# ooowedyn/InkLayer

Hardware: AMD Instinct MI355X
Metric: sketches/sec end-to-end (GroundingDINO+SAM) at 1024x1024 (higher is better)
Workload: dtype f16 (MFMA, f32 accumulate; f32 residual/norm/softmax; split-f16 = fp32-grade operands for patch-embed, neck, mask decoder)

## Files before the change

inklayer_amd/csrc/gemm.hip:

```cpp
#include <stdlib.h>

#include "common.h"
#include "../../include/inklayer_hip.h"

namespace {

template <int BK> struct Swz;
template <> struct Swz<64> {
  static __device__ __forceinline__ int f(int row) { return row & 7; }
};
template <> struct Swz<32> {
  static __device__ __forceinline__ int f(int row) { return (-(row >> 2)) & 3; }
};

typedef __attribute__((address_space(1))) const void* gptr_t;
typedef __attribute__((address_space(3))) void* lptr_t;

__device__ __forceinline__ bool residual_preloaded(const InkGemm& p) {
  return (p.residual || p.res_hi) && p.act == INK_ACT_NONE && !p.col_scale;
}

template <int TM>
__device__ __forceinline__ void wave_rows(int (&rows)[TM], const InkGemm& p, int mw, int lane) {
#pragma unroll
  for (int ti = 0; ti < TM; ++ti) {
    const int m = mw + ti * 16 + (lane & 15);
    int r = -1;
    if (m < p.M) r = p.row_map ? p.row_map[m] : m;
    rows[ti] = r;
  }
}

template <int TM, int TN, bool SPLIT = false>
__device__ __forceinline__ void init_wave_tile(f32x4 (&acc)[TM][TN], const InkGemm& p, const int (&rows)[TM], int nw,
                                               int lane) {
  const int fq = lane >> 4;
  const bool pre = residual_preloaded(p);
  if (SPLIT) {
#pragma unroll
    for (int ti = 0; ti < TM; ++ti) {
      const int r = pre ? rows[ti] : -1;
      const size_t off = (size_t)max(r, 0) * p.ldr + nw + fq * 4;
#pragma unroll
      for (int j = 0; j < TN; ++j) {
        acc[ti][j] = (f32x4){0.f, 0.f, 0.f, 0.f};
        if (r >= 0 && nw + j * 16 + fq * 4 < p.N) {
          const f16x4 h = *(const f16x4*)((const f16*)p.res_hi + off + j * 16);
          const f16x4 l = *(const f16x4*)((const f16*)p.res_lo + off + j * 16);
          acc[ti][j] = (f32x4){(float)h[0] + (float)l[0], (float)h[1] + (float)l[1], (float)h[2] + (float)l[2],
                               (float)h[3] + (float)l[3]};
        }
      }
    }
    return;
  }
#pragma unroll
  for (int ti = 0; ti < TM; ++ti) {
    const int r = pre ? rows[ti] : -1;
    const float* rp = p.residual + (size_t)max(r, 0) * p.ldr + nw + fq * 4;
#pragma unroll
    for (int j = 0; j < TN; ++j) {
      acc[ti][j] = (f32x4){0.f, 0.f, 0.f, 0.f};
      if (r >= 0 && nw + j * 16 + fq * 4 < p.N) acc[ti][j] = *(const f32x4*)(rp + j * 16);
    }
  }
}

template <int TM, int TN>
__device__ __forceinline__ void ln_rows_prologue(const InkGemm& p, float2* strip, int mw, int nw, int lane) {
  float2* cols = strip + TM * 16;
  for (int c = lane; c < TN * 16; c += 64) {
    const int n = nw + c;
    cols[c] = n < p.N ? make_float2(p.ln_colsum[n], p.bias ? p.bias[n] : 0.f) : make_float2(0.f, 0.f);
  }
  constexpr int RPL = (TM * 16 + 63) / 64;
  f32x4 v[RPL][10];
#pragma unroll
  for (int q = 0; q < RPL; ++q) {
    const int r = lane + 64 * q, m = mw + r;
    const f32x4* sp = (const f32x4*)((const float2*)p.ln_stats + (size_t)min(m, p.M - 1) * p.ln_parts);
#pragma unroll
    for (int k = 0; k < 10; ++k) v[q][k] = 2 * k < p.ln_parts ? sp[k] : (f32x4){0.f, 0.f, 0.f, 0.f};
  }
#pragma unroll
  for (int q = 0; q < RPL; ++q) {
    const int r = lane + 64 * q;
    double s1 = 0.0, s2 = 0.0;
#pragma unroll
    for (int k = 0; k < 10; ++k) {
      s1 += (double)v[q][k][0] + (double)v[q][k][2];
      s2 += (double)v[q][k][1] + (double)v[q][k][3];
    }
    const double mean = s1 / (double)p.ln_dim;
    const double var = fmax(s2 / (double)p.ln_dim - mean * mean, 0.0);
    const float rstd = (float)(1.0 / sqrt(var + (double)p.ln_eps));
    if (r < TM * 16) strip[r] = mw + r < p.M ? make_float2(rstd, rstd * (float)mean) : make_float2(0.f, 0.f);
  }
}

template <int TM, int TN>
__device__ __forceinline__ void add_bias_wave_tile(f32x4 (&acc)[TM][TN], const InkGemm& p, int nw, int lane) {
  const int fq = lane >> 4;
#pragma unroll
  for (int j = 0; j < TN; ++j) {
    const int n = nw + j * 16 + fq * 4;
    f32x4 bv = (f32x4){0.f, 0.f, 0.f, 0.f};
    if (p.bias && n < p.N) bv = *(const f32x4*)(p.bias + n);
#pragma unroll
    for (int ti = 0; ti < TM; ++ti) acc[ti][j] += bv;
  }
}

template <int TM, int TN, int OUT, int MODE = -1, bool LNF = false>
__device__ __forceinline__ void store_wave_tile(f32x4 (&acc)[TM][TN], const InkGemm& p, char* er,
                                                const int (&rows)[TM], int nw, int lane, const float2* strip = nullptr) {
  constexpr bool F16O = OUT == 1;
  constexpr int WNC = TN * 16, EP = WNC * 4 + 16;
  constexpr int ES = OUT == 0 ? 4 : 8;
  constexpr int CPRW = WNC / ES;
  constexpr int NIT = (16 * CPRW + 63) / 64;
  const int fr = lane & 15, fq = lane >> 4;
  const bool wide16 = OUT != 0 && (p.ldc % 8 == 0);
  const bool res_late = MODE < 0 && p.residual && !residual_preloaded(p);
  const int act = MODE < 0 ? p.act : MODE;
  const bool scaled = MODE < 0 && p.col_scale != nullptr;
  int row_of[NIT], n_of[NIT];
#pragma unroll
  for (int it = 0; it < NIT; ++it) {
    const int c = it * 64 + lane;
    row_of[it] = c < 16 * CPRW ? c / CPRW : 16;
    n_of[it] = nw + (c % CPRW) * ES;
  }

  if (LNF) {
    const float2* cols = strip + TM * 16;
#pragma unroll
    for (int j = 0; j < TN; ++j) {
      const f32x4 c01 = *(const f32x4*)(cols + j * 16 + fq * 4);
      const f32x4 c23 = *(const f32x4*)(cols + j * 16 + fq * 4 + 2);
      const f32x4 sv = (f32x4){c01[0], c01[2], c23[0], c23[2]}, bv = (f32x4){c01[1], c01[3], c23[1], c23[3]};
#pragma unroll
      for (int ti = 0; ti < TM; ++ti) {
        const float2 mr = strip[ti * 16 + fr];
#pragma unroll
        for (int e = 0; e < 4; ++e) acc[ti][j][e] = fmaf(mr.x, acc[ti][j][e], fmaf(-mr.y, sv[e], bv[e]));
      }
      __builtin_amdgcn_sched_barrier(0);
    }
  } else {
    add_bias_wave_tile<TM, TN>(acc, p, nw, lane);
  }

#pragma unroll
  for (int ti = 0; ti < TM; ++ti) {
    float s1 = 0.f, s2 = 0.f;
#pragma unroll
    for (int j = 0; j < TN; ++j) {
      f32x4 v = acc[ti][j];
      if (act == INK_ACT_GELU) {
#pragma unroll
        for (int r = 0; r < 4; ++r) v[r] = gelu_erf(v[r]);
      } else if (act == INK_ACT_RELU) {
#pragma unroll
        for (int r = 0; r < 4; ++r) v[r] = fmaxf(v[r], 0.f);
      }
      if (scaled) {
        const int n = nw + j * 16 + fq * 4;
        if (n < p.N) v *= *(const f32x4*)(p.col_scale + n);
      }
      if (OUT == 2 && nw + j * 16 + fq * 4 < p.N) {
        s1 += (v[0] + v[1]) + (v[2] + v[3]);
        s2 += (v[0] * v[0] + v[1] * v[1]) + (v[2] * v[2] + v[3] * v[3]);
      }
      if (F16O) {
        *(f16x4*)(er + fr * EP + (j * 16 + fq * 4) * 2) = (f16x4){(f16)v[0], (f16)v[1], (f16)v[2], (f16)v[3]};
      } else {
        *(f32x4*)(er + fr * EP + (j * 16 + fq * 4) * 4) = v;
      }
    }
    if (OUT == 2 && p.stats_out) {
      s1 += __shfl_xor(s1, 16, 64);
      s2 += __shfl_xor(s2, 16, 64);
      s1 += __shfl_xor(s1, 32, 64);
      s2 += __shfl_xor(s2, 32, 64);
      if (fq == 0 && rows[ti] >= 0)
        ((float2*)p.stats_out)[(size_t)rows[ti] * p.stats_parts + nw / WNC] = make_float2(s1, s2);
    }
#pragma unroll
    for (int it = 0; it < NIT; ++it) {
      int r = __builtin_amdgcn_ds_bpermute((row_of[it] & 15) << 2, rows[ti]);
      if (row_of[it] >= 16 || n_of[it] >= p.N) r = -1;
      if (r >= 0) {
        const int c_n = n_of[it];
        const char* src = er + row_of[it] * EP + (c_n - nw) * (F16O ? 2 : 4);
        if (F16O) {
          f16x8 d = *(const f16x8*)src;
          f16* dst = (f16*)p.C + (size_t)r * p.ldc + c_n;
          if (res_late) {
            const float* rp = p.residual + (size_t)r * p.ldr + c_n;
#pragma unroll
            for (int e = 0; e < 8; ++e)
              if (c_n + e < p.N) d[e] = (f16)((float)d[e] + rp[e]);
          }
          if (wide16 && c_n + 8 <= p.N) {
            *(f16x8*)dst = d;
          } else {
            *(f16x4*)dst = (f16x4){d[0], d[1], d[2], d[3]};
            if (c_n + 8 <= p.N) *(f16x4*)(dst + 4) = (f16x4){d[4], d[5], d[6], d[7]};
          }
        } else if (OUT == 2) {
          const f32x4 d0 = *(const f32x4*)src, d1 = *(const f32x4*)(src + 16);
          f16x8 hi, lo;
#pragma unroll
          for (int e = 0; e < 4; ++e) {
            hi[e] = (f16)d0[e];
            lo[e] = (f16)(d0[e] - (float)hi[e]);
            hi[e + 4] = (f16)d1[e];
            lo[e + 4] = (f16)(d1[e] - (float)hi[e + 4]);
          }
          f16* dh = (f16*)p.C + (size_t)r * p.ldc + c_n;
          f16* dl = (f16*)p.C_lo + (size_t)r * p.ldc + c_n;
          if (wide16 && c_n + 8 <= p.N) {
            *(f16x8*)dh = hi;
            *(f16x8*)dl = lo;
          } else {
            *(f16x4*)dh = (f16x4){hi[0], hi[1], hi[2], hi[3]};
            *(f16x4*)dl = (f16x4){lo[0], lo[1], lo[2], lo[3]};
            if (c_n + 8 <= p.N) {
              *(f16x4*)(dh + 4) = (f16x4){hi[4], hi[5], hi[6], hi[7]};
              *(f16x4*)(dl + 4) = (f16x4){lo[4], lo[5], lo[6], lo[7]};
            }
          }
        } else {
          f32x4 d = *(const f32x4*)src;
          if (res_late) d += *(const f32x4*)(p.residual + (size_t)r * p.ldr + c_n);
          *(f32x4*)((float*)p.C + (size_t)r * p.ldc + c_n) = d;
        }
      }
    }
  }
}

__device__ __forceinline__ void tile_of(int id, int ntm, int ntn, int group_m, int& mt, int& nt) {
  if (group_m > 1) {
    const int per = group_m * ntn;
    const int first = (id / per) * group_m;
    const int gsz = min(ntm - first, group_m);
    mt = first + (id % per) % gsz;
    nt = (id % per) / gsz;
  } else {
    mt = id / ntn;
    nt = id % ntn;
  }
}

constexpr int NS = 2;
template <int BM, int BN, int BK, int WM, int WN, bool EXT>
__global__ __launch_bounds__(WM * WN * 64) void gemm_f16_nt(InkGemm p, int group_m) {
  constexpr int NT = WM * WN * 64;
  constexpr int CPR = BK / 8;
  constexpr int ROWB = BK * 2;
  constexpr int TILE_A = BM * ROWB, TILE_W = BN * ROWB;
  constexpr int STAGE = TILE_A + TILE_W;
  constexpr int IT_A = (BM * CPR) / NT, IT_W = (BN * CPR) / NT;
  constexpr int TM = BM / WM / 16, TN = BN / WN / 16;
  static_assert((BM * CPR) % NT == 0 && (BN * CPR) % NT == 0, "tile/threads mismatch");
  extern __shared__ __attribute__((aligned(16))) char smem[];

  const int tid = threadIdx.x;
  const int lane = tid & 63;
  const int wave = tid >> 6;
  const int wm = wave / WN, wn = wave % WN;

  const int ntn = (p.N + BN - 1) / BN;
  const int ntm = (p.M + BM - 1) / BM;
  int mt, nt;
  tile_of(xcd_remap(blockIdx.x, ntm * ntn), ntm, ntn, group_m, mt, nt);
  const int m0 = mt * BM;
  const int n0 = nt * BN;

  const f16* __restrict__ A = (const f16*)p.A;
  const f16* __restrict__ W = (const f16*)p.W;

  const f16* srcA[IT_A];
  const f16* srcW[IT_W];
#pragma unroll
  for (int it = 0; it < IT_A; ++it) {
    const int pch = it * NT + tid;
    const int row = pch / CPR;
    const int lch = (pch % CPR) ^ Swz<BK>::f(row);
    srcA[it] = A + (size_t)min(m0 + row, p.M - 1) * p.lda + lch * 8;
  }
#pragma unroll
  for (int it = 0; it < IT_W; ++it) {
    const int pch = it * NT + tid;
    const int row = pch / CPR;
    const int lch = (pch % CPR) ^ Swz<BK>::f(row);
    srcW[it] = W + (size_t)min(n0 + row, p.N - 1) * p.ldw + lch * 8;
  }

  auto stage = [&](int buf, int kt) {
    char* base = smem + buf * STAGE;
#pragma unroll
    for (int it = 0; it < IT_A; ++it)
      __builtin_amdgcn_global_load_lds((gptr_t)(srcA[it] + kt * BK), (lptr_t)(base + (it * NT + wave * 64) * 16), 16, 0, 0);
#pragma unroll
    for (int it = 0; it < IT_W; ++it)
      __builtin_amdgcn_global_load_lds((gptr_t)(srcW[it] + kt * BK), (lptr_t)(base + TILE_A + (it * NT + wave * 64) * 16), 16, 0, 0);
  };

  int rows[TM];
  wave_rows<TM>(rows, p, m0 + wm * (BM / WM), lane);
  f32x4 acc[TM][TN];
  float2* strip = (float2*)(smem + NS * STAGE) + wave * (TM * 16 + TN * 16);
  if (EXT && p.ln_stats) ln_rows_prologue<TM, TN>(p, strip, m0 + wm * (BM / WM), n0 + wn * (BN / WN), lane);

  const int fr = lane & 15, fq = lane >> 4;
  const int offA = (wm * (BM / WM) + fr) * ROWB;
  const int offW = (wn * (BN / WN) + fr) * ROWB;
  const int swz = Swz<BK>::f(fr);

  const int nk = p.K / BK;
  auto compute = [&](int cur) {
    const char* bA = smem + cur * STAGE;
    const char* bW = bA + TILE_A;
#pragma unroll
    for (int kk = 0; kk < BK / 32; ++kk) {
      constexpr int AG = TM > 4 ? 4 : TM;
      f16x8 a[AG], w[TN];
      const int co = ((kk * 4 + fq) ^ swz) << 4;
#pragma unroll
      for (int j = 0; j < TN; ++j) w[j] = *(const f16x8*)(bW + offW + j * 16 * ROWB + co);
#pragma unroll
      for (int i0 = 0; i0 < TM; i0 += AG) {
#pragma unroll
        for (int i = 0; i < AG; ++i) a[i] = *(const f16x8*)(bA + offA + (i0 + i) * 16 * ROWB + co);
#pragma unroll
        for (int i = 0; i < AG; ++i)
#pragma unroll
          for (int j = 0; j < TN; ++j)
            acc[i0 + i][j] = __builtin_amdgcn_mfma_f32_16x16x32_f16(w[j], a[i], acc[i0 + i][j], 0, 0, 0);
      }
    }
  };

  stage(0, 0);
  if (EXT && p.res_hi) {
    init_wave_tile<TM, TN, true>(acc, p, rows, n0 + wn * (BN / WN), lane);
  } else {
    init_wave_tile<TM, TN>(acc, p, rows, n0 + wn * (BN / WN), lane);
  }
  for (int kt = 0; kt < nk; ++kt) {
    asm volatile("s_waitcnt vmcnt(0)" ::: "memory");
    __syncthreads();
    if (kt + 1 < nk) stage((kt + 1) & 1, kt + 1);
    compute(kt & 1);
  }

  constexpr int WNC = BN / WN;
  constexpr int EP = WNC * 4 + 16;
  static_assert(WM * WN * 16 * EP <= NS * STAGE, "epilogue patch must fit in the staging LDS");
  __syncthreads();
  char* er = smem + wave * (16 * EP);
  if (EXT && p.ln_stats) {
    if (p.c_f16 == 1) {
      store_wave_tile<TM, TN, 1, -1, true>(acc, p, er, rows, n0 + wn * WNC, lane, strip);
    } else {
      store_wave_tile<TM, TN, 0, -1, true>(acc, p, er, rows, n0 + wn * WNC, lane, strip);
    }
  } else if (EXT && p.c_f16 == 2) {
    store_wave_tile<TM, TN, 2>(acc, p, er, rows, n0 + wn * WNC, lane);
  } else if (p.c_f16 == 1) {
    store_wave_tile<TM, TN, 1>(acc, p, er, rows, n0 + wn * WNC, lane);
  } else {
    store_wave_tile<TM, TN, 0>(acc, p, er, rows, n0 + wn * WNC, lane);
  }
}

constexpr int PP_RING = 4, PP_TN = 5;
template <int EPI>
__global__ __launch_bounds__(512) void gemm_f16_nt_pp(InkGemm p, int group_m) {
  constexpr int RING = PP_RING, TN = PP_TN;
  constexpr int BM = 256, BN = 64 * TN, BK = 32, NT = 512;
  constexpr int CPR = BK / 8, ROWB = BK * 2;
  constexpr int TILE_A = BM * ROWB, TILE_W = BN * ROWB, GRAN = TILE_A + TILE_W;
  constexpr int IT_A = (BM * CPR) / NT, IT_W = (BN * CPR) / NT;
  constexpr bool W_TAIL = (BN * CPR) % NT != 0;
  static_assert(!W_TAIL || (BN * CPR) % NT == NT / 2, "tail is exactly the first four waves");
  constexpr int LOADS = IT_A + IT_W;
  constexpr int TM = 8, WNC = 16 * TN;
  constexpr int AHEAD = RING - 2;
  constexpr int AG = 4;
  constexpr int EP = WNC * 4 + 16;
  static_assert(8 * 16 * EP <= RING * GRAN, "patch fits");
  extern __shared__ __attribute__((aligned(16))) char smem[];
  const int tid = threadIdx.x, lane = tid & 63;
  const int wave = __builtin_amdgcn_readfirstlane(tid >> 6);
  const int grp = wave >> 2, wn = wave & 3;
  const int fr = lane & 15, fq = lane >> 4;

  const int ntn = (p.N + BN - 1) / BN, ntm = (p.M + BM - 1) / BM;
  int mt, nt;
  tile_of(xcd_remap(blockIdx.x, ntm * ntn), ntm, ntn, group_m, mt, nt);
  const int m0 = mt * BM, n0 = nt * BN;
  const int G = p.K / BK;
  const f16* __restrict__ A = (const f16*)p.A;
  const f16* __restrict__ W = (const f16*)p.W;
  const f16* srcA[IT_A];
  const f16* srcW[IT_W + (W_TAIL ? 1 : 0)];
#pragma unroll
  for (int it = 0; it < IT_A; ++it) {
    const int pch = it * NT + tid, row = pch / CPR, lch = (pch % CPR) ^ Swz<BK>::f(row);
    srcA[it] = A + (size_t)min(m0 + row, p.M - 1) * p.lda + lch * 8;
  }
#pragma unroll
  for (int it = 0; it < IT_W + (W_TAIL ? 1 : 0); ++it) {
    const int pch = it * NT + tid, row = min(pch / CPR, BN - 1), lch = (pch % CPR) ^ Swz<BK>::f(row);
    srcW[it] = W + (size_t)min(n0 + row, p.N - 1) * p.ldw + lch * 8;
  }
  auto dma = [&](int g, int slot) {
    char* base = smem + slot * GRAN;
#pragma unroll
    for (int it = 0; it < IT_A; ++it)
      __builtin_amdgcn_global_load_lds((gptr_t)(srcA[it] + g * BK), (lptr_t)(base + (it * NT + wave * 64) * 16), 16, 0, 0);
#pragma unroll
    for (int it = 0; it < IT_W; ++it)
      __builtin_amdgcn_global_load_lds((gptr_t)(srcW[it] + g * BK), (lptr_t)(base + TILE_A + (it * NT + wave * 64) * 16), 16, 0, 0);
    if (W_TAIL && grp == 0)
      __builtin_amdgcn_global_load_lds((gptr_t)(srcW[IT_W] + g * BK), (lptr_t)(base + TILE_A + (IT_W * NT + wave * 64) * 16), 16, 0, 0);
  };
  auto wait_ahead = [&]() {
    if (W_TAIL && grp == 0) {
      asm volatile("s_waitcnt vmcnt(%0)" ::"n"((AHEAD - 1) * (LOADS + 1)) : "memory");
    } else {
      asm volatile("s_waitcnt vmcnt(%0)" ::"n"((AHEAD - 1) * LOADS) : "memory");
    }
  };
  auto slot_end = [&]() {
    __builtin_amdgcn_sched_barrier(0);
    __builtin_amdgcn_s_barrier();
    __builtin_amdgcn_sched_barrier(0);
  };

  int rows[TM];
  wave_rows<TM>(rows, p, m0 + grp * 128, lane);
  float2* strip = (float2*)(smem + RING * GRAN) + wave * (128 + WNC);
#pragma unroll
  for (int g = 0; g < AHEAD; ++g) dma(g, g);
  if (EPI == 1 || EPI == 2) ln_rows_prologue<TM, TN>(p, strip, m0 + grp * 128, n0 + wn * WNC, lane);
  f32x4 acc[TM][TN];
  init_wave_tile<TM, TN, EPI == 3>(acc, p, rows, n0 + wn * WNC, lane);
  if (residual_preloaded(p) || EPI == 1 || EPI == 2) {
    asm volatile("s_waitcnt vmcnt(0)" ::: "memory");
  } else {
    wait_ahead();
  }
  slot_end();
  if (grp == 1) slot_end();

  const int offA = (grp * 128 + fr) * ROWB;
  const int offW = (wn * WNC + fr) * ROWB;
  const int co = (fq ^ Swz<BK>::f(fr)) << 4;
  f16x8 a[AG], w[TN];
  int cslot = 0, islot = AHEAD % RING;
  auto iter = [&](int g) __attribute__((always_inline)) {
    const char* bA = smem + cslot * GRAN;
    const char* bW = bA + TILE_A;
#pragma unroll
    for (int i = 0; i < AG; ++i) a[i] = *(const f16x8*)(bA + offA + i * 16 * ROWB + co);
#pragma unroll
    for (int j = 0; j < TN; ++j) w[j] = *(const f16x8*)(bW + offW + j * 16 * ROWB + co);
    if (g + AHEAD < G) {
      dma(g + AHEAD, islot);
      wait_ahead();
    } else {
      asm volatile("s_waitcnt vmcnt(0)" ::: "memory");
    }
    slot_end();
    asm volatile("s_waitcnt lgkmcnt(0)" ::: "memory");
    __builtin_amdgcn_sched_barrier(0);
    __builtin_amdgcn_s_setprio(1);
#pragma unroll
    for (int i0 = 0; i0 < TM; i0 += AG) {
#pragma unroll
      for (int i = 0; i < AG; ++i) {
#pragma unroll
        for (int j = 0; j < TN; ++j)
          acc[i0 + i][j] = __builtin_amdgcn_mfma_f32_16x16x32_f16(w[j], a[i], acc[i0 + i][j], 0, 0, 0);
        if (i0 + AG < TM) {
          a[i] = *(const f16x8*)(bA + offA + (i0 + AG + i) * 16 * ROWB + co);
          __builtin_amdgcn_sched_barrier(0);
        }
      }
    }
    __builtin_amdgcn_s_setprio(0);
    slot_end();
    cslot = (cslot + 1 == RING) ? 0 : cslot + 1;
    islot = (islot + 1 == RING) ? 0 : islot + 1;
  };
  for (int g = 0; g < G; ++g) iter(g);
  if (grp == 0) slot_end();

  char* er = smem + wave * (16 * EP);
  const bool plain = !p.col_scale && !(p.residual && !residual_preloaded(p));
  if constexpr (EPI == 1) {
    store_wave_tile<TM, TN, 1, INK_ACT_NONE, true>(acc, p, er, rows, n0 + wn * WNC, lane, strip);
  } else if constexpr (EPI == 2) {
    store_wave_tile<TM, TN, 1, INK_ACT_GELU, true>(acc, p, er, rows, n0 + wn * WNC, lane, strip);
  } else if constexpr (EPI == 3) {
    store_wave_tile<TM, TN, 2, INK_ACT_NONE>(acc, p, er, rows, n0 + wn * WNC, lane);
  } else if (p.c_f16) {
    if (plain && p.act == INK_ACT_GELU) {
      store_wave_tile<TM, TN, 1, INK_ACT_GELU>(acc, p, er, rows, n0 + wn * WNC, lane);
    } else if (plain && p.act == INK_ACT_NONE) {
      store_wave_tile<TM, TN, 1, INK_ACT_NONE>(acc, p, er, rows, n0 + wn * WNC, lane);
    } else {
      store_wave_tile<TM, TN, 1>(acc, p, er, rows, n0 + wn * WNC, lane);
    }
  } else {
    if (plain && p.act == INK_ACT_NONE) {
      store_wave_tile<TM, TN, 0, INK_ACT_NONE>(acc, p, er, rows, n0 + wn * WNC, lane);
    } else {
      store_wave_tile<TM, TN, 0>(acc, p, er, rows, n0 + wn * WNC, lane);
    }
  }
}

template <int EPI>
static int launch_gemm_pp(const InkGemm& p, hipStream_t s, int group_m) {
  if (p.K / 32 < PP_RING) return INK_ERR_ARG;
  if (EPI == 0 && (p.ln_stats || p.c_f16 == 2 || p.res_hi)) return INK_ERR_ARG;
  constexpr int BN = 64 * PP_TN;
  constexpr int lds = PP_RING * (256 + BN) * 32 * 2 + 8 * (128 + 16 * PP_TN) * 8;
  static_assert(lds <= 160 * 1024, "LDS budget");
  static bool attr = ((void)hipFuncSetAttribute((const void*)gemm_f16_nt_pp<EPI>,
                                                hipFuncAttributeMaxDynamicSharedMemorySize, lds), true);
  (void)attr;
  const int ntiles = ((p.M + 255) / 256) * ((p.N + BN - 1) / BN);
  hipLaunchKernelGGL((gemm_f16_nt_pp<EPI>), dim3(ntiles), dim3(512), lds, s, p, group_m);
  return ink_launch_status();
}

template <int BM, int BN, int BK, int WM, int WN, bool EXT>
static int launch_gemm(const InkGemm& p, hipStream_t s, int group_m = 1) {
  constexpr int lds = NS * (BM + BN) * BK * 2 + (EXT ? (BM * WN + BN * WM) * 8 : 0);
  static_assert(lds <= 160 * 1024, "LDS budget");
  if (!EXT && (p.ln_stats || p.c_f16 == 2 || p.res_hi)) return INK_ERR_ARG;
  static bool attr = ((void)hipFuncSetAttribute((const void*)gemm_f16_nt<BM, BN, BK, WM, WN, EXT>,
                                                hipFuncAttributeMaxDynamicSharedMemorySize, lds), true);
  (void)attr;
  const int ntm = (p.M + BM - 1) / BM, ntn = (p.N + BN - 1) / BN;
  hipLaunchKernelGGL((gemm_f16_nt<BM, BN, BK, WM, WN, EXT>), dim3(ntm * ntn), dim3(WM * WN * 64), lds, s, p, group_m);
  return ink_launch_status();
}

}

static int g_variant = -1;
extern "C" int ink_gemm_query_variant(int32_t M, int32_t N, int32_t K) {
  if (K % 64 != 0) return 32;
  if (N % 320 == 0 && K >= 128 && (long)((M + 255) / 256) * (N / 320) >= 384) return 45;
  const long tiles256 = (long)((M + 255) / 256) * ((N + 255) / 256);
  const bool n_fits = (N % 256 == 0) || N >= 1024;
  return (tiles256 >= 200 && n_fits) ? 10 : 0;
}
extern "C" int ink_gemm_query_stats_chunk(int32_t M, int32_t N, int32_t K) {
  return (K % 64 == 0 && ink_gemm_query_variant(M, N, K) == 45) ? 80 : 64;
}
extern "C" int ink_abi_version(void) { return INK_ABI_VERSION; }
extern "C" int ink_gemm_set_variant(int32_t v) {
  INK_CHECK_ARG(v == -1 || v == 0 || v == 10 || v == 45);
  g_variant = v;
  return INK_OK;
}

extern "C" int ink_gemm_f16(const InkGemm* pp, void* stream) {
  INK_CHECK_ARG(pp != nullptr);
  const InkGemm& p = *pp;
  INK_CHECK_ARG(p.A && p.W && p.C);
  INK_CHECK_ARG(p.M > 0 && p.N > 0 && p.K > 0);
  INK_CHECK_ARG(p.K % 32 == 0 && p.N % 4 == 0);
  INK_CHECK_ARG(p.lda % 8 == 0 && p.ldw % 8 == 0 && p.lda >= p.K && p.ldw >= p.K);
  INK_CHECK_ARG(p.ldc % 4 == 0 && p.ldc >= p.N);
  INK_CHECK_ARG(!p.residual || (p.ldr % 4 == 0 && p.ldr >= p.N));
  INK_CHECK_ARG(((uintptr_t)p.A & 15) == 0 && ((uintptr_t)p.W & 15) == 0);
  INK_CHECK_ARG(((uintptr_t)p.C & 15) == 0);
  INK_CHECK_ARG(p.act >= 0 && p.act <= 2);
  INK_CHECK_ARG(p.c_f16 >= 0 && p.c_f16 <= 2 && (p.c_f16 != 2 || (p.C_lo && ((uintptr_t)p.C_lo & 15) == 0)));
  INK_CHECK_ARG(!p.res_hi || !p.col_scale);
  INK_CHECK_ARG(!p.res_hi || (p.res_lo && !p.residual && p.ldr % 4 == 0 && p.ldr >= p.N && p.act == INK_ACT_NONE));
  INK_CHECK_ARG(!p.ln_stats || (p.ln_colsum && p.ln_parts > 0 && p.ln_parts <= 20 && p.ln_parts % 2 == 0 &&
                                p.ln_dim > 0 && !p.row_map && ((uintptr_t)p.ln_stats & 15) == 0));
  hipStream_t s = (hipStream_t)stream;
  const bool ext = p.ln_stats || p.c_f16 == 2 || p.res_hi;
  if (p.K % 64 != 0) return launch_gemm<128, 128, 32, 2, 2, true>(p, s);
  int v = g_variant;
  if (v < 0) {
    v = ink_gemm_query_variant(p.M, p.N, p.K);
    if (ext && v == 10) v = 0;
  }
  if (p.stats_out) {
    const bool pp3 = v == 45 && !p.ln_stats && !p.col_scale && !p.row_map && p.res_hi && p.act == INK_ACT_NONE;
    const int chunk = pp3 ? 80 : 64;
    INK_CHECK_ARG(p.c_f16 == 2 && p.N % chunk == 0 && p.stats_parts == p.N / chunk && g_variant < 0);
  }
  switch (v) {
    case 10: return launch_gemm<256, 256, 64, 4, 4, false>(p, s, 4);
    case 45:
      if (ext) {
        const bool simple = !p.col_scale && !p.row_map;
        if (p.ln_stats && p.c_f16 == 1 && simple && !p.residual && !p.res_hi && p.act == INK_ACT_NONE)
          return launch_gemm_pp<1>(p, s, 4);
        if (p.ln_stats && p.c_f16 == 1 && simple && !p.residual && !p.res_hi && p.act == INK_ACT_GELU)
          return launch_gemm_pp<2>(p, s, 4);
        if (!p.ln_stats && p.c_f16 == 2 && simple && p.res_hi && p.act == INK_ACT_NONE)
          return launch_gemm_pp<3>(p, s, 4);
        return launch_gemm<128, 128, 64, 2, 2, true>(p, s);
      }
      return launch_gemm_pp<0>(p, s, 4);
    default: return launch_gemm<128, 128, 64, 2, 2, true>(p, s);
  }
}
```

Before: 120.1.

## Add deeper multi-stage LDS ring and shape-based tile selection for generic GEMM

Generalizes the generic f16 GEMM kernel from a fixed double buffer to an NS-deep LDS ring, with partial vmcnt waits so loads for up to two future K-tiles stay in flight. It also adds a tile chooser that picks smaller tiles (64x64 or 32x64, 4-deep ring) when few 128x128 workgroups would launch, and a 4-deep ring for mid-size grids. The aim is to hide global-load latency and fill the GPU on small GEMMs. In exchange it uses more LDS per workgroup, which can lower occupancy, and the small tiles give less operand reuse.

```diff
diff --git a/inklayer_amd/csrc/gemm.hip b/inklayer_amd/csrc/gemm.hip
--- a/inklayer_amd/csrc/gemm.hip
+++ b/inklayer_amd/csrc/gemm.hip
@@ -254,9 +254,21 @@
   }
 }
 
-constexpr int NS = 2;
-template <int BM, int BN, int BK, int WM, int WN, bool EXT>
+template <int L, int NS>
+__device__ __forceinline__ void wait_dma_tiles(int ahead) {
+  static_assert((NS - 2) * L <= 63, "vmcnt is a 6-bit counter");
+  if (NS >= 4 && ahead == 2) {
+    asm volatile("s_waitcnt vmcnt(%0)" ::"n"(2 * L) : "memory");
+  } else if (NS >= 3 && ahead == 1) {
+    asm volatile("s_waitcnt vmcnt(%0)" ::"n"(L) : "memory");
+  } else {
+    asm volatile("s_waitcnt vmcnt(0)" ::: "memory");
+  }
+}
+
+template <int BM, int BN, int BK, int WM, int WN, bool EXT, int NS>
 __global__ __launch_bounds__(WM * WN * 64) void gemm_f16_nt(InkGemm p, int group_m) {
+  static_assert(NS >= 2 && NS <= 4, "ring depth");
   constexpr int NT = WM * WN * 64;
   constexpr int CPR = BK / 8;
   constexpr int ROWB = BK * 2;
@@ -344,17 +356,26 @@
     }
   };
 
-  stage(0, 0);
+#pragma unroll
+  for (int q = 0; q < NS - 1; ++q)
+    if (q < nk) stage(q, q);
   if (EXT && p.res_hi) {
     init_wave_tile<TM, TN, true>(acc, p, rows, n0 + wn * (BN / WN), lane);
   } else {
     init_wave_tile<TM, TN>(acc, p, rows, n0 + wn * (BN / WN), lane);
   }
+  if (residual_preloaded(p)) asm volatile("s_waitcnt vmcnt(0)" ::: "memory");
+  int cslot = 0, islot = NS - 1;
   for (int kt = 0; kt < nk; ++kt) {
-    asm volatile("s_waitcnt vmcnt(0)" ::: "memory");
-    __syncthreads();
-    if (kt + 1 < nk) stage((kt + 1) & 1, kt + 1);
-    compute(kt & 1);
+    wait_dma_tiles<IT_A + IT_W, NS>(min(NS - 2, nk - 1 - kt));
+    asm volatile("s_waitcnt lgkmcnt(0)" ::: "memory");
+    __builtin_amdgcn_sched_barrier(0);
+    __builtin_amdgcn_s_barrier();
+    __builtin_amdgcn_sched_barrier(0);
+    if (kt + NS - 1 < nk) stage(islot, kt + NS - 1);
+    compute(cslot);
+    cslot = cslot + 1 == NS ? 0 : cslot + 1;
+    islot = islot + 1 == NS ? 0 : islot + 1;
   }
 
   constexpr int WNC = BN / WN;
@@ -541,17 +562,36 @@
   return ink_launch_status();
 }
 
-template <int BM, int BN, int BK, int WM, int WN, bool EXT>
+template <int BM, int BN, int BK, int WM, int WN, bool EXT, int NS>
 static int launch_gemm(const InkGemm& p, hipStream_t s, int group_m = 1) {
   constexpr int lds = NS * (BM + BN) * BK * 2 + (EXT ? (BM * WN + BN * WM) * 8 : 0);
   static_assert(lds <= 160 * 1024, "LDS budget");
   if (!EXT && (p.ln_stats || p.c_f16 == 2 || p.res_hi)) return INK_ERR_ARG;
-  static bool attr = ((void)hipFuncSetAttribute((const void*)gemm_f16_nt<BM, BN, BK, WM, WN, EXT>,
+  static bool attr = ((void)hipFuncSetAttribute((const void*)gemm_f16_nt<BM, BN, BK, WM, WN, EXT, NS>,
                                                 hipFuncAttributeMaxDynamicSharedMemorySize, lds), true);
   (void)attr;
   const int ntm = (p.M + BM - 1) / BM, ntn = (p.N + BN - 1) / BN;
-  hipLaunchKernelGGL((gemm_f16_nt<BM, BN, BK, WM, WN, EXT>), dim3(ntm * ntn), dim3(WM * WN * 64), lds, s, p, group_m);
+  hipLaunchKernelGGL((gemm_f16_nt<BM, BN, BK, WM, WN, EXT, NS>), dim3(ntm * ntn), dim3(WM * WN * 64), lds, s, p, group_m);
   return ink_launch_status();
+}
+
+enum GemmTile {
+  T128_R2, T128_R4,
+  T64_R4, T32X64_R4,
+  T128K32_R2,
+  T256_R2,
+};
+
+static int launch_tile(int t, const InkGemm& p, hipStream_t s) {
+  switch (t) {
+    case T128_R2: return launch_gemm<128, 128, 64, 2, 2, true, 2>(p, s);
+    case T128_R4: return launch_gemm<128, 128, 64, 2, 2, true, 4>(p, s);
+    case T64_R4: return launch_gemm<64, 64, 64, 2, 2, true, 4>(p, s);
+    case T32X64_R4: return launch_gemm<32, 64, 64, 1, 4, true, 4>(p, s);
+    case T128K32_R2: return launch_gemm<128, 128, 32, 2, 2, true, 2>(p, s);
+    case T256_R2: return launch_gemm<256, 256, 64, 4, 4, false, 2>(p, s, 4);
+    default: return INK_ERR_ARG;
+  }
 }
 
 }
@@ -572,6 +612,17 @@
   INK_CHECK_ARG(v == -1 || v == 0 || v == 10 || v == 45);
   g_variant = v;
   return INK_OK;
+}
+
+static int choose_tile(const InkGemm& p, int v) {
+  if (v == 32) return T128K32_R2;
+  if (v == 10) return T256_R2;
+  const long wg128 = (long)((p.M + 127) / 128) * ((p.N + 127) / 128);
+  if (!p.stats_out && wg128 < 128) {
+    const long wg64 = (long)((p.M + 63) / 64) * ((p.N + 63) / 64);
+    return wg64 >= 128 ? T64_R4 : T32X64_R4;
+  }
+  return (wg128 <= 256 && p.K / 64 >= 3) ? T128_R4 : T128_R2;
 }
 
 extern "C" int ink_gemm_f16(const InkGemm* pp, void* stream) {
@@ -593,7 +644,7 @@
                                 p.ln_dim > 0 && !p.row_map && ((uintptr_t)p.ln_stats & 15) == 0));
   hipStream_t s = (hipStream_t)stream;
   const bool ext = p.ln_stats || p.c_f16 == 2 || p.res_hi;
-  if (p.K % 64 != 0) return launch_gemm<128, 128, 32, 2, 2, true>(p, s);
+  if (p.K % 64 != 0) return launch_tile(choose_tile(p, 32), p, s);
   int v = g_variant;
   if (v < 0) {
     v = ink_gemm_query_variant(p.M, p.N, p.K);
@@ -605,7 +656,7 @@
     INK_CHECK_ARG(p.c_f16 == 2 && p.N % chunk == 0 && p.stats_parts == p.N / chunk && g_variant < 0);
   }
   switch (v) {
-    case 10: return launch_gemm<256, 256, 64, 4, 4, false>(p, s, 4);
+    case 10: return launch_tile(choose_tile(p, 10), p, s);
     case 45:
       if (ext) {
         const bool simple = !p.col_scale && !p.row_map;
@@ -615,9 +666,9 @@
           return launch_gemm_pp<2>(p, s, 4);
         if (!p.ln_stats && p.c_f16 == 2 && simple && p.res_hi && p.act == INK_ACT_NONE)
           return launch_gemm_pp<3>(p, s, 4);
-        return launch_gemm<128, 128, 64, 2, 2, true>(p, s);
+        return launch_tile(choose_tile(p, 0), p, s);
       }
       return launch_gemm_pp<0>(p, s, 4);
-    default: return launch_gemm<128, 128, 64, 2, 2, true>(p, s);
-  }
-}
+    default: return launch_tile(choose_tile(p, 0), p, s);
+  }
+}
```

After: 120.7 (median of 6 runs). Within noise of the previous version (+0.6%).
